# urw7rs/diffusion-models-made-easy

Hardware: AMD Instinct MI355X
Metric: denoising steps/sec + training images/sec, DDPM UNet CIFAR10 32×32 @1/2/4/8 GPU (higher is better)
Workload: dtype bf16; 1 GPU; DDPM T=1000 sampling, CIFAR10 32x32, default UNet (32,416,643 params, random init), batch 128 per GPU, t.shape=(1,); global_batch=128, parallelism=dp1 (independent chains per GPU, no data-path collective)

## Files before the change

diffusion-models-made-easy_amd/csrc/conv_thin.hip:

```cpp
#include <stdio.h>

#include <type_traits>

#include "conv_common.h"

namespace dmme {

constexpr int kThinMaxC = 512;

template <int NT, typename T = bf16, bool SPLIT = false>
__global__ void __launch_bounds__(256) conv_out_thin_kernel(ConvArgs a, int R) {
    typedef typename Vec8<T>::type bf16x8;
    extern __shared__ __attribute__((aligned(16))) char lds[];
    const int C = a.C1, W = a.Wout, H = a.Hout, NCOL = a.Cout * 9;
    float* par = reinterpret_cast<float*>(lds);
    float* z = par + 2 * C;
    constexpr int ZP = 32 * NT + 1;
    const int tid = threadIdx.x, lane = tid & 63, wave = tid >> 6;
    const int r = lane & 31, h = lane >> 5;
    const int bands = H / R, n = blockIdx.x / bands, y0 = (blockIdx.x % bands) * R;
    const int npx = (R + 2) * W, ntile = npx / 32;

    const int ksteps = C / 16;
    const T* wb = (const T*)a.w;
    bf16x8 wfrag[NT][8];
    bf16x8 wlo[SPLIT ? NT : 1][SPLIT ? 8 : 1];
    auto load_w = [&](int kc) __attribute__((always_inline)) {
#pragma unroll
        for (int t = 0; t < NT; ++t) {
            const int nc = 32 * t + r;
#pragma unroll
            for (int kg = 0; kg < 8; ++kg) {
                bf16x8 v, vl;
#pragma unroll
                for (int e = 0; e < 8; ++e) v[e] = vl[e] = (T)0.f;
                if constexpr (SPLIT) {
                    const int c0 = (kc + kg) * 16 + 8 * h;
                    if (kc + kg < ksteps && nc < NCOL) {
                        const T* wr = wb + (int64_t)nc * 2 * C + (c0 >> 5) * 64 + (c0 & 31);
                        v = *reinterpret_cast<const bf16x8*>(wr);
                        vl = *reinterpret_cast<const bf16x8*>(wr + 32);
                    }
                    wlo[t][kg] = vl;
                } else {
                    if (kc + kg < ksteps && nc < NCOL) v = *reinterpret_cast<const bf16x8*>(wb + (int64_t)nc * C + (kc + kg) * 16 + 8 * h);
                }
                wfrag[t][kg] = v;
            }
        }
    };
    const bool w_once = ksteps <= 8;
    if (w_once) load_w(0);
    for (int c = tid; c < C; c += 256) {
        float sc = 1.f, sh = 0.f;
        if (a.has_gni) {
            gn_in_scale_shift(a, n, c, C, y0 == 0, sc, sh);
        } else if (a.scale) {
            sc = a.scale[(int64_t)n * C + c];
            sh = a.shift[(int64_t)n * C + c];
        }
        par[c] = sc;
        par[C + c] = sh;
    }
    __syncthreads();

    typedef typename std::conditional<SPLIT, float, T>::type TX;
    const TX* xb = (const TX*)a.src1 + (int64_t)n * H * W * C;
    for (int tile = wave; tile < ntile; tile += 4) {
        const int p = tile * 32 + r;
        const int yy = y0 - 1 + p / W, xx = p % W;
        const bool in = yy >= 0 && yy < H;
        const TX* px = xb + (int64_t)((in ? yy : 0) * W + xx) * C + 8 * h;
        f32x16 acc[NT];
#pragma unroll
        for (int t = 0; t < NT; ++t)
#pragma unroll
            for (int j = 0; j < 16; ++j) acc[t][j] = 0.f;
        for (int kc = 0; kc < ksteps; kc += 8) {
            if (!w_once) load_w(kc);
            if constexpr (SPLIT) {
                uint4 raw[8][2];
#pragma unroll
                for (int kg = 0; kg < 8; ++kg)
                    if (kc + kg < ksteps) {
                        raw[kg][0] = *reinterpret_cast<const uint4*>(px + (kc + kg) * 16);
                        raw[kg][1] = *reinterpret_cast<const uint4*>(px + (kc + kg) * 16 + 4);
                    }
#pragma unroll
                for (int kg = 0; kg < 8; ++kg) {
                    if (kc + kg >= ksteps) break;
                    const int c0 = (kc + kg) * 16 + 8 * h;
                    bf16x8 ahi, alo;
#pragma unroll
                    for (int q = 0; q < 2; ++q) {
                        f32x4 y = __builtin_bit_cast(f32x4, raw[kg][q]);
                        if (a.scale) {
                            const f32x4 sc4 = *reinterpret_cast<const f32x4*>(par + c0 + 4 * q), sh4 = *reinterpret_cast<const f32x4*>(par + C + c0 + 4 * q);
#pragma unroll
                            for (int e = 0; e < 4; ++e) y[e] = fmaf(y[e], sc4[e], sh4[e]);
                        }
                        if (a.pro_silu) {
#pragma unroll
                            for (int e = 0; e < 4; ++e) y[e] = silu_fast(y[e]);
                        }
#pragma unroll
                        for (int e = 0; e < 4; ++e) {
                            const T hv = (T)(in ? y[e] : 0.f);
                            ahi[4 * q + e] = hv;
                            alo[4 * q + e] = (T)((in ? y[e] : 0.f) - (float)hv);
                        }
                    }
#pragma unroll
                    for (int t = 0; t < NT; ++t) {
                        mma16<T>(__builtin_bit_cast(uint4, alo), __builtin_bit_cast(uint4, wfrag[t][kg]), acc[t]);
                        mma16<T>(__builtin_bit_cast(uint4, ahi), __builtin_bit_cast(uint4, wlo[t][kg]), acc[t]);
                        mma16<T>(__builtin_bit_cast(uint4, ahi), __builtin_bit_cast(uint4, wfrag[t][kg]), acc[t]);
                    }
                }
            } else {
            uint4 raw[8];
#pragma unroll
            for (int kg = 0; kg < 8; ++kg)
                if (kc + kg < ksteps) raw[kg] = *reinterpret_cast<const uint4*>(px + (kc + kg) * 16);
#pragma unroll
            for (int kg = 0; kg < 8; ++kg) {
                if (kc + kg >= ksteps) break;
                const int c0 = (kc + kg) * 16 + 8 * h;
                uint4 av = prologue_vec<T>(raw[kg], a.scale ? par + c0 : nullptr, a.scale ? par + C + c0 : nullptr, nullptr, a.pro_silu);
                if (!in) av = make_uint4(0u, 0u, 0u, 0u);
#pragma unroll
                for (int t = 0; t < NT; ++t) mma16<T>(av, __builtin_bit_cast(uint4, wfrag[t][kg]), acc[t]);
            }
            }
        }
#pragma unroll
        for (int t = 0; t < NT; ++t)
#pragma unroll
            for (int j = 0; j < 16; ++j) z[(tile * 32 + (j & 3) + 8 * (j >> 2) + 4 * h) * ZP + 32 * t + r] = acc[t][j];
    }
    __syncthreads();
    const int hw = H * W;
    float* out = (float*)a.dst + (int64_t)n * a.Cout * hw;
    for (int q = tid; q < R * W; q += 256) {
        const int oy = q / W, ox = q % W;
        for (int k = 0; k < a.Cout; ++k) {
            float s = a.bias ? a.bias[k] : 0.f;
#pragma unroll
            for (int t9 = 0; t9 < 9; ++t9) {
                const int xs = ox + t9 % 3 - 1;
                if (xs < 0 || xs >= W) continue;
                s += z[((oy + t9 / 3) * W + xs) * ZP + k * 9 + t9];
            }
            out[(int64_t)k * hw + (y0 + oy) * W + ox] = s;
        }
    }
}

static int thin_rows(const ConvArgs& a) {
    const int NT = a.Cout * 9 <= 32 ? 1 : 2;
    const size_t cap = (a.mix == 3 ? 80 : 60) * 1024;
    for (int R = 16; R >= 2; R >>= 1)
        if (a.Hout % R == 0 && ((R + 2) * a.Wout) % 32 == 0 && (size_t)(R + 2) * a.Wout * (32 * NT + 1) * 4 + (size_t)2 * a.C1 * 4 <= cap &&
            (int64_t)a.N * (a.Hout / R) >= 512)
            return R;
    for (int R = 2; R <= 16; R <<= 1)
        if (a.Hout % R == 0 && ((R + 2) * a.Wout) % 32 == 0 && (size_t)(R + 2) * a.Wout * (32 * NT + 1) * 4 + (size_t)2 * a.C1 * 4 <= cap) return R;
    return 0;
}

bool conv_thin_route(int dtype, const ConvArgs& a, ConvRoute& r) {
    const bool off = getenv("DMME_NO_CONV_THIN") != nullptr;
    if (a.mix && a.mix != 3) return false;
    if (off || !is16(dtype) || a.x3) return false;
    if (a.mix == 3 && (dtype != DMME_F16 || a.C1 % 32)) return false;
    if (a.taps != 9 || a.stride != 1 || a.up || a.C2 || a.in_nchw || !a.out_nchw || a.out_silu || a.tproj || a.res1 || a.dmask || a.gn_part || a.n_gno)
        return false;
    if (a.Cout * 9 > 64 || a.C1 % 16 || a.C1 > kThinMaxC || a.Wout % 32 || a.Hin != a.Hout || a.Win != a.Wout) return false;
    if (thin_rows(a) <= 0) return false;
    r = make_route(CONV_THIN);
    return true;
}

int launch_conv_out_thin(const ConvArgs& a, hipStream_t s) {
    const int R = thin_rows(a);
    DMME_REQUIRE(R > 0, DMME_ERR_UNSUPPORTED, "conv_out_thin: unsupported shape");
    const int NT = a.Cout * 9 <= 32 ? 1 : 2;
    const size_t lds = (size_t)(R + 2) * a.Wout * (32 * NT + 1) * 4 + (size_t)2 * a.C1 * 4;
    const dim3 grid((unsigned)(a.N * (a.Hout / R)));
    if (a.mix == 3) {
        static bool attr = false;
        if (!attr) {
            DMME_CHECK_HIP(hipFuncSetAttribute(reinterpret_cast<const void*>(conv_out_thin_kernel<1, f16, true>), hipFuncAttributeMaxDynamicSharedMemorySize, 80 * 1024));
            DMME_CHECK_HIP(hipFuncSetAttribute(reinterpret_cast<const void*>(conv_out_thin_kernel<2, f16, true>), hipFuncAttributeMaxDynamicSharedMemorySize, 80 * 1024));
            attr = true;
        }
        if (NT == 1)
            hipLaunchKernelGGL((conv_out_thin_kernel<1, f16, true>), grid, dim3(256), lds, s, a, R);
        else
            hipLaunchKernelGGL((conv_out_thin_kernel<2, f16, true>), grid, dim3(256), lds, s, a, R);
    } else if (a.f16) {
        if (NT == 1)
            hipLaunchKernelGGL((conv_out_thin_kernel<1, f16>), grid, dim3(256), lds, s, a, R);
        else
            hipLaunchKernelGGL((conv_out_thin_kernel<2, f16>), grid, dim3(256), lds, s, a, R);
    } else if (NT == 1)
        hipLaunchKernelGGL((conv_out_thin_kernel<1, bf16>), grid, dim3(256), lds, s, a, R);
    else
        hipLaunchKernelGGL((conv_out_thin_kernel<2, bf16>), grid, dim3(256), lds, s, a, R);
    DMME_CHECK_LAUNCH();
    return DMME_OK;
}

}
```

diffusion-models-made-easy_amd/csrc/kernels_generic.hip:

```cpp
#include <stdlib.h>

#include <algorithm>

#include "common.h"

namespace dmme {

template <typename T>
__global__ void __launch_bounds__(256) conv_generic_kernel(ConvArgs a) {
    const int64_t total = (int64_t)a.N * a.Hout * a.Wout * a.Cout;
    const int Cin = a.C1 + a.C2;
    const int Hv = a.up ? 2 * a.Hin : a.Hin, Wv = a.up ? 2 * a.Win : a.Win;
    const int k = a.taps == 9 ? 3 : 1, pad = a.taps == 9 ? 1 : 0;
    for (int64_t idx = blockIdx.x * (int64_t)blockDim.x + threadIdx.x; idx < total;
         idx += (int64_t)gridDim.x * blockDim.x) {
        const int co = (int)(idx % a.Cout);
        int64_t p = idx / a.Cout;
        const int ow = (int)(p % a.Wout);
        p /= a.Wout;
        const int oh = (int)(p % a.Hout);
        const int n = (int)(p / a.Hout);
        const T* w = (const T*)a.w + (int64_t)co * a.taps * Cin;
        const float* sc = a.scale ? a.scale + (int64_t)n * Cin : nullptr;
        const float* sh = a.scale ? a.shift + (int64_t)n * Cin : nullptr;
        const float* dm = a.dmask ? a.dmask + (int64_t)n * Cin : nullptr;
        float acc = 0.f;
        for (int kh = 0; kh < k; ++kh) {
            const int iy = oh * a.stride - pad + kh;
            if (iy < 0 || iy >= Hv) continue;
            if (a.up == 2 && (iy & 1)) continue;
            const int sy = a.up ? (iy >> 1) : iy;
            for (int kw = 0; kw < k; ++kw) {
                const int ix = ow * a.stride - pad + kw;
                if (ix < 0 || ix >= Wv) continue;
                if (a.up == 2 && (ix & 1)) continue;
                const int sx = a.up ? (ix >> 1) : ix;
                const T* wt = w + (kh * k + kw) * Cin;
                const int64_t pix = ((int64_t)n * a.Hin + sy) * a.Win + sx;
                for (int ci = 0; ci < Cin; ++ci) {
                    float v;
                    if (a.in_nchw)
                        v = ((const float*)a.src1)[(((int64_t)n * a.C1 + ci) * a.Hin + sy) * a.Win + sx];
                    else if (ci < a.C1)
                        v = to_f(((const T*)a.src1)[pix * a.C1 + ci]);
                    else
                        v = to_f(((const T*)a.src2)[pix * a.C2 + (ci - a.C1)]);
                    if (sc) v = fmaf(v, sc[ci], sh[ci]);
                    if (a.pro_silu) v = silu_f(v);
                    if (dm) v *= dm[ci];
                    if (!a.in_nchw) v = to_f(from_f<T>(v));
                    acc = fmaf(v, to_f(wt[ci]), acc);
                }
            }
        }
        if (a.bias) acc += a.bias[co];
        if (a.tproj) acc += a.tproj[(int64_t)(a.nt == 1 ? 0 : n) * a.tproj_ld + co];
        const int64_t opix = ((int64_t)n * a.Hout + oh) * a.Wout + ow;
        if (a.res1) {
            if (co < a.R1)
                acc += to_f(((const T*)a.res1)[opix * a.R1 + co]);
            else
                acc += to_f(((const T*)a.res2)[opix * (a.Cout - a.R1) + (co - a.R1)]);
        }
        if (a.out_silu) acc = silu_f(acc);
        if (a.out_nchw)
            ((float*)a.dst)[(((int64_t)n * a.Cout + co) * a.Hout + oh) * a.Wout + ow] = acc;
        else
            ((T*)a.dst)[opix * a.Cout + co] = from_f<T>(acc);
    }
}

template <typename T>
__global__ void __launch_bounds__(256) conv_in_kernel(ConvArgs a, int px_per_block) {
    extern __shared__ __attribute__((aligned(16))) float wl[];
    const int Cin = a.C1, K = 9 * Cin, Cout = a.Cout;
    for (int e = threadIdx.x; e < K * Cout; e += blockDim.x) {
        const int co = e / K, k = e % K;
        wl[k * Cout + co] = to_f(((const T*)a.w)[e]);
    }
    __syncthreads();
    const int tpp = Cout / 8;
    const int ppb = 256 / tpp;
    const int cg = (threadIdx.x % tpp) * 8;
    const int64_t npix = (int64_t)a.N * a.Hout * a.Wout;
    const int64_t p0 = (int64_t)blockIdx.x * px_per_block;
    for (int pp = threadIdx.x / tpp; pp < px_per_block; pp += ppb) {
        const int64_t p = p0 + pp;
        if (p >= npix) break;
        const int ox = (int)(p % a.Wout), oy = (int)((p / a.Wout) % a.Hout), n = (int)(p / ((int64_t)a.Wout * a.Hout));
        float acc[8];
#pragma unroll
        for (int j = 0; j < 8; ++j) acc[j] = a.bias ? a.bias[cg + j] : 0.f;
        for (int kh = 0; kh < 3; ++kh) {
            const int iy = oy - 1 + kh;
            if (iy < 0 || iy >= a.Hin) continue;
            for (int kw = 0; kw < 3; ++kw) {
                const int ix = ox - 1 + kw;
                if (ix < 0 || ix >= a.Win) continue;
                for (int ci = 0; ci < Cin; ++ci) {
                    const float v = a.in_nchw ? ((const float*)a.src1)[(((int64_t)n * Cin + ci) * a.Hin + iy) * a.Win + ix]
                                              : to_f(((const T*)a.src1)[(((int64_t)n * a.Hin + iy) * a.Win + ix) * Cin + ci]);
                    const float* wr = wl + ((kh * 3 + kw) * Cin + ci) * Cout + cg;
                    const float4 w0 = *reinterpret_cast<const float4*>(wr), w1 = *reinterpret_cast<const float4*>(wr + 4);
                    acc[0] = fmaf(v, w0.x, acc[0]); acc[1] = fmaf(v, w0.y, acc[1]);
                    acc[2] = fmaf(v, w0.z, acc[2]); acc[3] = fmaf(v, w0.w, acc[3]);
                    acc[4] = fmaf(v, w1.x, acc[4]); acc[5] = fmaf(v, w1.y, acc[5]);
                    acc[6] = fmaf(v, w1.z, acc[6]); acc[7] = fmaf(v, w1.w, acc[7]);
                }
            }
        }
        T* o = (T*)a.dst + p * Cout + cg;
#pragma unroll
        for (int j = 0; j < 8; ++j) o[j] = from_f<T>(acc[j]);
    }
}

typedef float f32x16_g __attribute__((ext_vector_type(16)));
typedef float f32x4_g __attribute__((ext_vector_type(4)));
template <typename T, int CT>
__global__ void __launch_bounds__(256) conv_in_mfma_kernel(ConvArgs a, int nblocks) {
    const int lane = threadIdx.x & 63, r = lane & 31, h = lane >> 5;
    const int Cin = a.C1, K = 9 * Cin;
    float wreg[CT][14];
#pragma unroll
    for (int ct = 0; ct < CT; ++ct)
#pragma unroll
        for (int j = 0; j < 14; ++j) {
            const int k = 2 * j + h;
            wreg[ct][j] = k < K ? to_f(((const T*)a.w)[(int64_t)(ct * 32 + r) * K + k]) : 0.f;
        }
    const int HW = a.Hout * a.Wout;
    int t_off[14], t_dy[14], t_dx[14];
#pragma unroll
    for (int j = 0; j < 14; ++j) {
        const int k = 2 * j + h, tap = k / Cin, ci = k - tap * Cin;
        t_dy[j] = k < K ? tap / 3 - 1 : 1 << 20;
        t_dx[j] = tap % 3 - 1;
        t_off[j] = (ci * a.Hin + (tap / 3 - 1)) * a.Win + tap % 3 - 1;
    }
    __shared__ __attribute__((aligned(16))) float biasL[128];
    if (threadIdx.x < 32 * CT) biasL[threadIdx.x] = a.bias ? a.bias[threadIdx.x] : 0.f;
    __syncthreads();
    for (int blk = blockIdx.x * 4 + (threadIdx.x >> 6); blk < nblocks; blk += gridDim.x * 4) {
        const int p = blk * 32 + r;
        const int n = p / HW, rem = p - n * HW, oy = rem / a.Wout, ox = rem - oy * a.Wout;
        const float* xb = (const float*)a.src1 + ((int64_t)n * Cin * a.Hin + oy) * a.Win + ox;
        float xv[14];
#pragma unroll
        for (int j = 0; j < 14; ++j) {
            const bool in = (unsigned)(oy + t_dy[j]) < (unsigned)a.Hin && (unsigned)(ox + t_dx[j]) < (unsigned)a.Win;
            xv[j] = in ? xb[t_off[j]] : 0.f;
        }
        constexpr int PITCH = CT * 32 + 4;
        __shared__ __attribute__((aligned(16))) unsigned short stage_in[4][32 * PITCH];
        unsigned short* st = stage_in[threadIdx.x >> 6];
#pragma unroll
        for (int ct = 0; ct < CT; ++ct) {
            f32x16_g acc;
#pragma unroll
            for (int g4 = 0; g4 < 4; ++g4) {
                const f32x4_g b4 = *reinterpret_cast<const f32x4_g*>(biasL + ct * 32 + 8 * g4 + 4 * h);
                acc[4 * g4] = b4[0];
                acc[4 * g4 + 1] = b4[1];
                acc[4 * g4 + 2] = b4[2];
                acc[4 * g4 + 3] = b4[3];
            }
#pragma unroll
            for (int j = 0; j < 14; ++j) acc = __builtin_amdgcn_mfma_f32_32x32x2f32(wreg[ct][j], xv[j], acc, 0, 0, 0);
            if constexpr (sizeof(T) == 2) {
#pragma unroll
                for (int gq = 0; gq < 4; ++gq) {
                    typedef T bf16x4_g __attribute__((ext_vector_type(4)));
                    bf16x4_g v;
#pragma unroll
                    for (int e = 0; e < 4; ++e) v[e] = (T)acc[4 * gq + e];
                    *reinterpret_cast<bf16x4_g*>(st + r * PITCH + ct * 32 + 8 * gq + 4 * h) = v;
                    if (a.gn_part) {
                        float s = 0.f, ss = 0.f;
#pragma unroll
                        for (int e = 0; e < 4; ++e) {
                            const float x = (float)v[e];
                            s += x;
                            ss = fmaf(x, x, ss);
                        }
                        s = half_sum(s);
                        ss = half_sum(ss);
                        if (r == 0) {
                            const float mean = s * (1.f / 128.f);
                            float* po = a.gn_part + (((int64_t)n * a.gn_tiles + (rem >> 5)) * (a.Cout / 4) + ct * 8 + 2 * gq + h) * 2;
                            po[0] = mean;
                            po[1] = ss - s * mean;
                        }
                    }
                }
            } else {
                T* o = (T*)a.dst + (int64_t)p * a.Cout + ct * 32 + 4 * h;
#pragma unroll
                for (int gq = 0; gq < 4; ++gq)
                    *reinterpret_cast<float4*>(o + 8 * gq) = make_float4(acc[4 * gq], acc[4 * gq + 1], acc[4 * gq + 2], acc[4 * gq + 3]);
                if (a.gn_part) {
#pragma unroll
                    for (int gq = 0; gq < 4; ++gq) {
                        float s = 0.f, ss = 0.f;
#pragma unroll
                        for (int e = 0; e < 4; ++e) {
                            const float x = acc[4 * gq + e];
                            s += x;
                            ss = fmaf(x, x, ss);
                        }
                        s = half_sum(s);
                        ss = half_sum(ss);
                        if (r == 0) {
                            const float mean = s * (1.f / 128.f);
                            float* po = a.gn_part + (((int64_t)n * a.gn_tiles + (rem >> 5)) * (a.Cout / 4) + ct * 8 + 2 * gq + h) * 2;
                            po[0] = mean;
                            po[1] = ss - s * mean;
                        }
                    }
                }
            }
        }
        if constexpr (sizeof(T) == 2) {
            __builtin_amdgcn_wave_barrier();
            constexpr int VPR = CT * 4;
#pragma unroll
            for (int q = 0; q < 32 * VPR / 64; ++q) {
                const int it = lane + 64 * q, px = it / VPR, sg = it % VPR;
                const uint2 lo = *reinterpret_cast<const uint2*>(st + px * PITCH + sg * 8), hi = *reinterpret_cast<const uint2*>(st + px * PITCH + sg * 8 + 4);
                *reinterpret_cast<uint4*>((T*)a.dst + (int64_t)(blk * 32 + px) * a.Cout + sg * 8) = make_uint4(lo.x, lo.y, hi.x, hi.y);
            }
            __builtin_amdgcn_wave_barrier();
        }
    }
}

static bool conv_in_mfma_supported(const ConvArgs& a) {
    return a.in_nchw && !a.out_nchw && a.taps == 9 && a.stride == 1 && !a.up && a.C2 == 0 && a.C1 <= 3 && !a.scale && !a.pro_silu && !a.dmask &&
           !a.tproj && !a.res1 && !a.out_silu && (a.Cout == 128 || a.Cout == 64 || a.Cout == 32) &&
           (!a.gn_part || (a.gn_cg == 4 && (a.Hout * a.Wout) % 32 == 0)) &&
           ((int64_t)a.N * a.Hout * a.Wout) % 32 == 0 && (int64_t)a.N * a.Hout * a.Wout * a.Cout < (1ll << 31) && !debug_route("no_conv_in_mfma");
}

void conv_generic_route(const ConvArgs& a, ConvRoute& r) {
    r = make_route(CONV_GENERIC);
    if (!conv_in_mfma_supported(a) || (a.Hout * a.Wout) % 32) return;
    r.vec = r.stat_bn = 4;
    r.stat_px = 32;
    r.stat_tiles = a.Hout * a.Wout / 32;
}

static bool conv_in_supported(const ConvArgs& a) {
    return !a.out_nchw && a.taps == 9 && a.stride == 1 && !a.up && a.C2 == 0 && a.C1 <= 8 && !a.scale &&
           !a.pro_silu && !a.dmask && !a.tproj && !a.res1 && !a.out_silu && a.Cout % 8 == 0 && a.Cout <= 2048 &&
           256 % (a.Cout / 8) == 0 && (size_t)9 * a.C1 * a.Cout * 4 <= 48 * 1024;
}

const char* conv_generic_kernel_name(const ConvArgs& a) {
    return conv_in_mfma_supported(a) ? "conv_in_mfma_kernel" : conv_in_supported(a) ? "conv_in_kernel" : "conv_generic_kernel";
}

int launch_conv_generic(int dtype, const ConvArgs& a, hipStream_t s) {
    if (conv_in_mfma_supported(a)) {
        const int nblocks = (int)((int64_t)a.N * a.Hout * a.Wout / 32);
        unsigned grid = (unsigned)((nblocks + 3) / 4);
        if (grid > 512u) grid = 512u;
#define DMME_CIN(TT, CT) hipLaunchKernelGGL((conv_in_mfma_kernel<TT, CT>), dim3(grid), dim3(256), 0, s, a, nblocks)
        if (dtype == DMME_BF16) {
            if (a.Cout == 128) DMME_CIN(bf16, 4); else if (a.Cout == 64) DMME_CIN(bf16, 2); else DMME_CIN(bf16, 1);
        } else if (dtype == DMME_F16) {
            if (a.Cout == 128) DMME_CIN(f16, 4); else if (a.Cout == 64) DMME_CIN(f16, 2); else DMME_CIN(f16, 1);
        } else {
            if (a.Cout == 128) DMME_CIN(float, 4); else if (a.Cout == 64) DMME_CIN(float, 2); else DMME_CIN(float, 1);
        }
#undef DMME_CIN
        DMME_CHECK_LAUNCH();
        return DMME_OK;
    }
    if (conv_in_supported(a) && !a.gn_part) {
        const int64_t npix = (int64_t)a.N * a.Hout * a.Wout;
        const int ppb = 256 / (a.Cout / 8) * 8;
        const unsigned blocks = (unsigned)((npix + ppb - 1) / ppb);
        const size_t lds = (size_t)9 * a.C1 * a.Cout * 4;
        if (dtype == DMME_BF16)
            hipLaunchKernelGGL(conv_in_kernel<bf16>, dim3(blocks), dim3(256), lds, s, a, ppb);
        else if (dtype == DMME_F16)
            hipLaunchKernelGGL(conv_in_kernel<f16>, dim3(blocks), dim3(256), lds, s, a, ppb);
        else
            hipLaunchKernelGGL(conv_in_kernel<float>, dim3(blocks), dim3(256), lds, s, a, ppb);
        DMME_CHECK_LAUNCH();
        return DMME_OK;
    }
    const int64_t total = (int64_t)a.N * a.Hout * a.Wout * a.Cout;
    if (total == 0) return DMME_OK;
    int64_t blocks = (total + 255) / 256;
    if (blocks > 65536) blocks = 65536;
    if (dtype == DMME_BF16)
        hipLaunchKernelGGL(conv_generic_kernel<bf16>, dim3((unsigned)blocks), dim3(256), 0, s, a);
    else if (dtype == DMME_F16)
        hipLaunchKernelGGL(conv_generic_kernel<f16>, dim3((unsigned)blocks), dim3(256), 0, s, a);
    else
        hipLaunchKernelGGL(conv_generic_kernel<float>, dim3((unsigned)blocks), dim3(256), 0, s, a);
    DMME_CHECK_LAUNCH();
    return DMME_OK;
}

template <typename T>
__global__ void __launch_bounds__(256) gn_generic_kernel(const T* __restrict__ s1, const T* __restrict__ s2, int HW,
                                                         int C1, int C2, int groups, const float* gamma,
                                                         const float* beta, float eps, float* scale, float* shift,
                                                         float* mean_rstd) {
    __shared__ float red[16];
    const int n = blockIdx.y, g = blockIdx.x;
    const int C = C1 + C2, cg = C / groups;
    const int64_t cnt = (int64_t)cg * HW;
    auto at = [&](int64_t e) -> float {
        const int c = g * cg + (int)(e % cg);
        const int64_t p = (int64_t)n * HW + e / cg;
        return c < C1 ? to_f(s1[p * C1 + c]) : to_f(s2[p * C2 + (c - C1)]);
    };
    float s = 0.f;
    for (int64_t e = threadIdx.x; e < cnt; e += blockDim.x) s += at(e);
    const float mean = block_sum(s, red) / (float)cnt;
    float q = 0.f;
    for (int64_t e = threadIdx.x; e < cnt; e += blockDim.x) {
        const float d = at(e) - mean;
        q = fmaf(d, d, q);
    }
    const float var = block_sum(q, red) / (float)cnt;
    const float rstd = 1.0f / sqrtf(var + eps);
    if (mean_rstd && threadIdx.x == 0) {
        mean_rstd[((int64_t)n * groups + g) * 2] = mean;
        mean_rstd[((int64_t)n * groups + g) * 2 + 1] = rstd;
    }
    for (int j = threadIdx.x; j < cg; j += blockDim.x) {
        const int c = g * cg + j;
        const float a = rstd * gamma[c];
        scale[(int64_t)n * C + c] = a;
        shift[(int64_t)n * C + c] = beta[c] - mean * a;
    }
}

int launch_gn_generic(int dtype, const void* src1, const void* src2, int N, int HW, int C1, int C2, int groups,
                      const float* gamma, const float* beta, float eps, float* scale, float* shift, float* mean_rstd,
                      hipStream_t s) {
    dim3 grid(groups, N);
    if (dtype == DMME_BF16)
        hipLaunchKernelGGL(gn_generic_kernel<bf16>, grid, dim3(256), 0, s, (const bf16*)src1, (const bf16*)src2, HW,
                           C1, C2, groups, gamma, beta, eps, scale, shift, mean_rstd);
    else if (dtype == DMME_F16)
        hipLaunchKernelGGL(gn_generic_kernel<f16>, grid, dim3(256), 0, s, (const f16*)src1, (const f16*)src2, HW,
                           C1, C2, groups, gamma, beta, eps, scale, shift, mean_rstd);
    else
        hipLaunchKernelGGL(gn_generic_kernel<float>, grid, dim3(256), 0, s, (const float*)src1, (const float*)src2,
                           HW, C1, C2, groups, gamma, beta, eps, scale, shift, mean_rstd);
    DMME_CHECK_LAUNCH();
    return DMME_OK;
}

template <typename T>
__global__ void __launch_bounds__(256) attn_generic_kernel(const T* __restrict__ qkv, int S, int C, int heads, int N, T* __restrict__ out) {
    extern __shared__ __attribute__((aligned(16))) float sm[];
    const int d = C / heads;
    float* qs = sm;
    float* ps = sm + d;
    float* red = ps + S;
    const int bh = blockIdx.y, n = bh / heads, hd = bh % heads, i = blockIdx.x;
    const T* base = qkv + (int64_t)n * S * 3 * C + (int64_t)hd * 3 * d;
    const float kscale = powf((float)C, -0.5f);
    for (int c = threadIdx.x; c < d; c += blockDim.x) qs[c] = to_f(base[(int64_t)i * 3 * C + c]);
    __syncthreads();
    float lmax = -INFINITY;
    for (int j = threadIdx.x; j < S; j += blockDim.x) {
        const T* kr = base + (int64_t)j * 3 * C + d;
        float acc = 0.f;
        for (int c = 0; c < d; ++c) acc = fmaf(qs[c], to_f(from_f<T>(to_f(kr[c]) * kscale)), acc);
        ps[j] = acc;
        lmax = fmaxf(lmax, acc);
    }
    const float m = block_max(lmax, red);
    float lsum = 0.f;
    for (int j = threadIdx.x; j < S; j += blockDim.x) {
        const float e = expf(ps[j] - m);
        ps[j] = e;
        lsum += e;
    }
    const float tot = block_sum(lsum, red);
    __syncthreads();
    const float inv = 1.0f / tot;
    const int on = bh % N, oh = bh / N;
    for (int c = threadIdx.x; c < d; c += blockDim.x) {
        float acc = 0.f;
        for (int j = 0; j < S; ++j) acc = fmaf(to_f(from_f<T>(ps[j] * inv)), to_f(base[(int64_t)j * 3 * C + 2 * d + c]), acc);
        out[((int64_t)on * S + i) * C + oh * d + c] = from_f<T>(acc);
    }
}

template <typename T>
__global__ void __launch_bounds__(256) attn_s16_kernel(const T* __restrict__ qkv, int C, int heads, int N, T* __restrict__ out) {
    extern __shared__ __attribute__((aligned(16))) float sm[];
    constexpr int S = 16;
    const int d = C / heads, dp = d + 4;
    float* qs = sm;
    float* ks = qs + S * dp;
    float* vs = ks + S * dp;
    float* ps = vs + S * dp;
    const int bh = blockIdx.x, n = bh / heads, hd = bh % heads, tid = threadIdx.x;
    const T* base = qkv + (int64_t)n * S * 3 * C + (int64_t)hd * 3 * d;
    const float kscale = powf((float)C, -0.5f);
    for (int e = tid; e < S * d; e += 256) {
        const int row = e / d, c = e - row * d;
        const T* p = base + (int64_t)row * 3 * C + c;
        qs[row * dp + c] = to_f(p[0]);
        ks[row * dp + c] = to_f(from_f<T>(to_f(p[d]) * kscale));
        vs[row * dp + c] = to_f(p[2 * d]);
    }
    __syncthreads();
    const int i = tid >> 4, j = tid & 15;
    float acc = 0.f;
    for (int c = 0; c < d; c += 4) {
        const f32x4_g a = *reinterpret_cast<const f32x4_g*>(qs + i * dp + c), b = *reinterpret_cast<const f32x4_g*>(ks + j * dp + c);
        acc = fmaf(a[0], b[0], acc);
        acc = fmaf(a[1], b[1], acc);
        acc = fmaf(a[2], b[2], acc);
        acc = fmaf(a[3], b[3], acc);
    }
    float m = acc;
    m = fmaxf(m, DMME_DPP_F(m, 0xB1));
    m = fmaxf(m, DMME_DPP_F(m, 0x4E));
    m = fmaxf(m, DMME_DPP_F(m, 0x141));
    m = fmaxf(m, DMME_DPP_F(m, 0x140));
    const float e = expf(acc - m);
    const float tot = row16_sum(e);
    ps[i * 17 + j] = to_f(from_f<T>(e * (1.0f / tot)));
    __syncthreads();
    const int on = bh % N, oh = bh / N;
    for (int c = j; c < d; c += 16) {
        float o = 0.f;
#pragma unroll
        for (int jj = 0; jj < S; ++jj) o = fmaf(ps[i * 17 + jj], vs[jj * dp + c], o);
        out[((int64_t)on * S + i) * C + oh * d + c] = from_f<T>(o);
    }
}

int launch_attn_heads(int dtype, const void* qkv, int N, int S, int C, int heads, void* out, hipStream_t s) {
    DMME_REQUIRE(heads >= 1 && C % heads == 0, DMME_ERR_INVALID, "attention: width %d not divisible by %d heads", C, heads);
    if (S == 16 && (C / heads) % 4 == 0 && C / heads <= 1024 && !debug_route("no_attn_s16")) {
        const size_t lds16 = (size_t)(3 * 16 * (C / heads + 4) + 16 * 17) * sizeof(float);
        if (lds16 <= 64 * 1024) {
            if (dtype == DMME_BF16)
                hipLaunchKernelGGL(attn_s16_kernel<bf16>, dim3((unsigned)(N * heads)), dim3(256), lds16, s, (const bf16*)qkv, C, heads, N, (bf16*)out);
            else if (dtype == DMME_F16)
                hipLaunchKernelGGL(attn_s16_kernel<f16>, dim3((unsigned)(N * heads)), dim3(256), lds16, s, (const f16*)qkv, C, heads, N, (f16*)out);
            else
                hipLaunchKernelGGL(attn_s16_kernel<float>, dim3((unsigned)(N * heads)), dim3(256), lds16, s, (const float*)qkv, C, heads, N, (float*)out);
            DMME_CHECK_LAUNCH();
            return DMME_OK;
        }
    }
    const size_t lds = (size_t)(C / heads + S + 16) * sizeof(float);
    DMME_REQUIRE(lds <= 64 * 1024, DMME_ERR_UNSUPPORTED, "attention generic: d+S too large (%d+%d)", C / heads, S);
    dim3 grid(S, N * heads);
    if (dtype == DMME_BF16)
        hipLaunchKernelGGL(attn_generic_kernel<bf16>, grid, dim3(256), lds, s, (const bf16*)qkv, S, C, heads, N, (bf16*)out);
    else if (dtype == DMME_F16)
        hipLaunchKernelGGL(attn_generic_kernel<f16>, grid, dim3(256), lds, s, (const f16*)qkv, S, C, heads, N, (f16*)out);
    else
        hipLaunchKernelGGL(attn_generic_kernel<float>, grid, dim3(256), lds, s, (const float*)qkv, S, C, heads, N, (float*)out);
    DMME_CHECK_LAUNCH();
    return DMME_OK;
}
int launch_attn_generic(int dtype, const void* qkv, int N, int S, int C, void* out, hipStream_t s) {
    return launch_attn_heads(dtype, qkv, N, S, C, 1, out, s);
}

__global__ void gn_modulate_kernel(float* __restrict__ scale, float* __restrict__ shift, const float* __restrict__ t_shift,
                                   const float* __restrict__ t_scale, int ld, int nt, int N, int C) {
    const int i = blockIdx.x * blockDim.x + threadIdx.x;
    if (i >= N * C) return;
    const int n = i / C, c = i % C, r = nt == 1 ? 0 : n;
    const float m = 1.0f + t_scale[(int64_t)r * ld + c];
    scale[i] = scale[i] * m;
    shift[i] = fmaf(shift[i], m, t_shift[(int64_t)r * ld + c]);
}
int launch_gn_modulate(float* scale, float* shift, const float* t_shift, const float* t_scale, int ld, int nt, int N, int C, hipStream_t s) {
    hipLaunchKernelGGL(gn_modulate_kernel, dim3((N * C + 255) / 256), dim3(256), 0, s, scale, shift, t_shift, t_scale, ld, nt, N, C);
    DMME_CHECK_LAUNCH();
    return DMME_OK;
}

__global__ void time_sinusoid_kernel(const int64_t* t, int nt, const float* freqs, int half, float* out, unsigned* mark, unsigned mark_val) {
    const int i = blockIdx.x * blockDim.x + threadIdx.x;
    if (i == 0 && mark) *mark = mark_val;
    if (i >= nt * half) return;
    const int r = i / half, k = i % half;
    const float arg = (float)t[r] * freqs[k];
    out[(int64_t)r * 2 * half + k] = sinf(arg);
    out[(int64_t)r * 2 * half + half + k] = cosf(arg);
}

int launch_time_sinusoid(const int64_t* t, int nt, const float* freqs, int half, float* out, hipStream_t s, unsigned* mark, unsigned mark_val) {
    const int total = nt * half;
    hipLaunchKernelGGL(time_sinusoid_kernel, dim3((total + 255) / 256), dim3(256), 0, s, t, nt, freqs, half, out, mark, mark_val);
    DMME_CHECK_LAUNCH();
    return DMME_OK;
}

__global__ void __launch_bounds__(256) label_cond_kernel(const float* z2, int nt, const float* __restrict__ E, const int64_t* __restrict__ labels, int K,
                                                         int emb, float* __restrict__ temb, float* zsave, int* status) {
    const int b = blockIdx.x;
    const int64_t y = labels[b];
    const bool ok = y >= 0 && y <= (int64_t)K;
    const int row = y < 0 ? 0 : (y > (int64_t)K ? K : (int)y);
    const float* zr = z2 + (int64_t)(nt == 1 ? 0 : b) * emb;
    const float* er = E + (int64_t)row * emb;
    for (int c = threadIdx.x; c < emb; c += blockDim.x) {
        const float v = zr[c] + er[c];
        if (zsave) zsave[(int64_t)b * emb + c] = v;
        temb[(int64_t)b * emb + c] = ok ? silu_f(v) : NAN;
    }
    if (!ok && threadIdx.x == 0 && status) atomicExch(status, 1);
}
int launch_label_cond(const float* z2, int nt, const float* E, const int64_t* labels, int B, int K, int emb, float* temb, float* zsave, int* status,
                      hipStream_t s) {
    DMME_REQUIRE(z2 && E && labels && temb && B > 0 && K >= 1 && emb > 0 && (nt == 1 || nt == B), DMME_ERR_INVALID, "label_cond: bad argument");
    DMME_REQUIRE(!zsave || zsave != z2 || nt == B, DMME_ERR_INVALID, "label_cond: in-place pre-activations need one time row per image");
    hipLaunchKernelGGL(label_cond_kernel, dim3((unsigned)B), dim3(256), 0, s, z2, nt, E, labels, K, emb, temb, zsave, status);
    DMME_CHECK_LAUNCH();
    return DMME_OK;
}

__global__ void __launch_bounds__(256) label_grad_kernel(const float* __restrict__ dz2, const int64_t* __restrict__ labels, int B, int emb,
                                                         float* __restrict__ dE) {
    __shared__ unsigned char hit[256];
    const int64_t k = blockIdx.x;
    const int tid = threadIdx.x;
    for (int c0 = 0; c0 < emb; c0 += 256) {
        const int c = c0 + tid;
// ... 573 lines not shown
```

Baseline: 469.6 denoising steps/s (one step = UNet forward + DDPM update on a batch of 128), summed over GPUs.

## Prefetch next input gather and stage conv_in weights through LDS

Restructures the first-layer conv MFMA kernel so each wave gathers the input pixels for its next block while computing the current one, giving a software-pipelined loop. Weights are now loaded with coalesced vector loads into shared memory and then scattered into registers, replacing strided per-thread global loads. Boundary checks use a precomputed tap bitmask. Optional compile-time clock-stamp instrumentation is also added to both kernels; it is disabled by default. The trade-off is higher register pressure from the double-buffered input and an extra barrier, and the shared buffer is reused for both weights and the output stage.

New measurement: 470.8 denoising steps/s (one step = UNet forward + DDPM update on a batch of 128), summed over GPUs (median of 6 runs). No clear change (+0.3%).

```diff
diff --git a/diffusion-models-made-easy_amd/csrc/conv_thin.hip b/diffusion-models-made-easy_amd/csrc/conv_thin.hip
--- a/diffusion-models-made-easy_amd/csrc/conv_thin.hip
+++ b/diffusion-models-made-easy_amd/csrc/conv_thin.hip
@@ -8,6 +8,13 @@
 
 constexpr int kThinMaxC = 512;
 
+#ifdef THIN_STAMPS
+#define THIN_STAMP() { __builtin_amdgcn_sched_barrier(0); if (stamping && st_i < 64) st_lds[st_i++] = (long long)clock64(); __builtin_amdgcn_sched_barrier(0); }
+#define THIN_STAMP_W() { __builtin_amdgcn_sched_barrier(0); __builtin_amdgcn_s_waitcnt(0); THIN_STAMP(); }
+#else
+#define THIN_STAMP()
+#define THIN_STAMP_W()
+#endif
 template <int NT, typename T = bf16, bool SPLIT = false>
 __global__ void __launch_bounds__(256) conv_out_thin_kernel(ConvArgs a, int R) {
     typedef typename Vec8<T>::type bf16x8;
@@ -50,6 +57,12 @@
         }
     };
     const bool w_once = ksteps <= 8;
+#ifdef THIN_STAMPS
+    __shared__ long long st_lds[64];
+    int st_i = 0;
+    const bool stamping = a.stamps && blockIdx.x == 0 && tid == 0;
+#endif
+    THIN_STAMP();
     if (w_once) load_w(0);
     for (int c = tid; c < C; c += 256) {
         float sc = 1.f, sh = 0.f;
@@ -63,6 +76,7 @@
         par[C + c] = sh;
     }
     __syncthreads();
+    THIN_STAMP();
 
     typedef typename std::conditional<SPLIT, float, T>::type TX;
     const TX* xb = (const TX*)a.src1 + (int64_t)n * H * W * C;
@@ -122,6 +136,7 @@
 #pragma unroll
             for (int kg = 0; kg < 8; ++kg)
                 if (kc + kg < ksteps) raw[kg] = *reinterpret_cast<const uint4*>(px + (kc + kg) * 16);
+            THIN_STAMP();
 #pragma unroll
             for (int kg = 0; kg < 8; ++kg) {
                 if (kc + kg >= ksteps) break;
@@ -133,12 +148,15 @@
             }
             }
         }
+        THIN_STAMP();
 #pragma unroll
         for (int t = 0; t < NT; ++t)
 #pragma unroll
             for (int j = 0; j < 16; ++j) z[(tile * 32 + (j & 3) + 8 * (j >> 2) + 4 * h) * ZP + 32 * t + r] = acc[t][j];
+        THIN_STAMP();
     }
     __syncthreads();
+    THIN_STAMP();
     const int hw = H * W;
     float* out = (float*)a.dst + (int64_t)n * a.Cout * hw;
     for (int q = tid; q < R * W; q += 256) {
@@ -154,7 +172,15 @@
             out[(int64_t)k * hw + (y0 + oy) * W + ox] = s;
         }
     }
-}
+    THIN_STAMP();
+    THIN_STAMP_W();
+#ifdef THIN_STAMPS
+    if (stamping)
+        for (int i = 0; i < st_i; ++i) a.stamps[i] = st_lds[i];
+#endif
+}
+#undef THIN_STAMP
+#undef THIN_STAMP_W
 
 static int thin_rows(const ConvArgs& a) {
     const int NT = a.Cout * 9 <= 32 ? 1 : 2;
diff --git a/diffusion-models-made-easy_amd/csrc/kernels_generic.hip b/diffusion-models-made-easy_amd/csrc/kernels_generic.hip
--- a/diffusion-models-made-easy_amd/csrc/kernels_generic.hip
+++ b/diffusion-models-made-easy_amd/csrc/kernels_generic.hip
@@ -117,43 +117,113 @@
 
 typedef float f32x16_g __attribute__((ext_vector_type(16)));
 typedef float f32x4_g __attribute__((ext_vector_type(4)));
+template <int CIN>
+__device__ __forceinline__ void cin_tap_table(int h, int Hin, int Win, int (&t_off)[14], int (&t_tap)[14]) {
+#pragma unroll
+    for (int j = 0; j < 14; ++j) {
+        int off[2], tp[2];
+#pragma unroll
+        for (int e = 0; e < 2; ++e) {
+            const int k = 2 * j + e, tap = k / CIN, ci = k % CIN;
+            off[e] = k < 9 * CIN ? (ci * Hin + (tap / 3 - 1)) * Win + tap % 3 - 1 : 0;
+            tp[e] = k < 9 * CIN ? tap : 31;
+        }
+        t_off[j] = h ? off[1] : off[0];
+        t_tap[j] = h ? tp[1] : tp[0];
+    }
+}
+#ifdef CIN_STAMPS
+#define CIN_STAMP() { __builtin_amdgcn_sched_barrier(0); if (stamping && st_i < 64) st_lds[st_i++] = (long long)clock64(); __builtin_amdgcn_sched_barrier(0); }
+#define CIN_STAMP_W() { __builtin_amdgcn_sched_barrier(0); __builtin_amdgcn_s_waitcnt(0); CIN_STAMP(); }
+#else
+#define CIN_STAMP()
+#define CIN_STAMP_W()
+#endif
 template <typename T, int CT>
 __global__ void __launch_bounds__(256) conv_in_mfma_kernel(ConvArgs a, int nblocks) {
     const int lane = threadIdx.x & 63, r = lane & 31, h = lane >> 5;
     const int Cin = a.C1, K = 9 * Cin;
-    float wreg[CT][14];
-#pragma unroll
-    for (int ct = 0; ct < CT; ++ct)
+    constexpr int PITCH = CT * 32 + 4;
+    constexpr int STAGE_BYTES = sizeof(T) == 2 ? 4 * 32 * PITCH * 2 : 0, W_BYTES = CT * 32 * 27 * (int)sizeof(T);
+    __shared__ __attribute__((aligned(16))) unsigned char smem[STAGE_BYTES > W_BYTES ? STAGE_BYTES : W_BYTES];
+    __shared__ __attribute__((aligned(16))) float biasL[128];
+#ifdef CIN_STAMPS
+    __shared__ long long st_lds[64];
+    int st_i = 0;
+    const bool stamping = a.stamps && blockIdx.x == 0 && threadIdx.x == 0;
+#endif
+    CIN_STAMP();
+    int t_off[14], t_tap[14];
+    if (Cin == 3) cin_tap_table<3>(h, a.Hin, a.Win, t_off, t_tap);
+    else if (Cin == 2) cin_tap_table<2>(h, a.Hin, a.Win, t_off, t_tap);
+    else cin_tap_table<1>(h, a.Hin, a.Win, t_off, t_tap);
+    const int HW = a.Hout * a.Wout;
+    auto gather = [&](int b, float (&x)[14], int& n_, int& rem_) __attribute__((always_inline)) {
+        const int p = b * 32 + r;
+        n_ = p / HW;
+        rem_ = p - n_ * HW;
+        const int oy = rem_ / a.Wout, ox = rem_ - oy * a.Wout;
+        const float* xb = (const float*)a.src1 + ((int64_t)n_ * Cin * a.Hin + oy) * a.Win + ox;
+        const unsigned cm = (ox > 0 ? 1u : 0u) | 2u | (ox + 1 < a.Win ? 4u : 0u);
+        const unsigned mask = (oy > 0 ? cm : 0u) | cm << 3 | (oy + 1 < a.Hin ? cm << 6 : 0u);
 #pragma unroll
         for (int j = 0; j < 14; ++j) {
-            const int k = 2 * j + h;
-            wreg[ct][j] = k < K ? to_f(((const T*)a.w)[(int64_t)(ct * 32 + r) * K + k]) : 0.f;
-        }
-    const int HW = a.Hout * a.Wout;
-    int t_off[14], t_dy[14], t_dx[14];
-#pragma unroll
-    for (int j = 0; j < 14; ++j) {
-        const int k = 2 * j + h, tap = k / Cin, ci = k - tap * Cin;
-        t_dy[j] = k < K ? tap / 3 - 1 : 1 << 20;
-        t_dx[j] = tap % 3 - 1;
-        t_off[j] = (ci * a.Hin + (tap / 3 - 1)) * a.Win + tap % 3 - 1;
-    }
-    __shared__ __attribute__((aligned(16))) float biasL[128];
+            const bool in = (mask >> t_tap[j]) & 1u;
+            const float v = xb[in ? t_off[j] : 0];
+            x[j] = in ? v : 0.f;
+        }
+    };
+    const int bstep = gridDim.x * 4;
+    int blk = blockIdx.x * 4 + (threadIdx.x >> 6);
+    float xv[14];
+    int n = 0, rem = 0;
+#pragma unroll
+    for (int j = 0; j < 14; ++j) xv[j] = 0.f;
+    if (blk < nblocks) gather(blk, xv, n, rem);
+    {
+        const T* wg = (const T*)a.w;
+        const int nw = CT * 32 * K;
+        if ((reinterpret_cast<uintptr_t>(wg) & 15) == 0) {
+            const int nv = nw * (int)sizeof(T) / 16;
+            constexpr int NIT = (W_BYTES / 16 + 255) / 256;
+            uint4 wv[NIT];
+#pragma unroll
+            for (int it = 0; it < NIT; ++it) {
+                const int v = threadIdx.x + 256 * it;
+                wv[it] = reinterpret_cast<const uint4*>(wg)[v < nv ? v : 0];
+            }
+#pragma unroll
+            for (int it = 0; it < NIT; ++it) {
+                const int v = threadIdx.x + 256 * it;
+                if (v < nv) reinterpret_cast<uint4*>(smem)[v] = wv[it];
+            }
+        } else {
+#pragma clang loop vectorize(disable) unroll(disable)
+            for (int e = threadIdx.x; e < nw; e += 256) reinterpret_cast<T*>(smem)[e] = wg[e];
+        }
+    }
     if (threadIdx.x < 32 * CT) biasL[threadIdx.x] = a.bias ? a.bias[threadIdx.x] : 0.f;
     __syncthreads();
-    for (int blk = blockIdx.x * 4 + (threadIdx.x >> 6); blk < nblocks; blk += gridDim.x * 4) {
-        const int p = blk * 32 + r;
-        const int n = p / HW, rem = p - n * HW, oy = rem / a.Wout, ox = rem - oy * a.Wout;
-        const float* xb = (const float*)a.src1 + ((int64_t)n * Cin * a.Hin + oy) * a.Win + ox;
-        float xv[14];
-#pragma unroll
-        for (int j = 0; j < 14; ++j) {
-            const bool in = (unsigned)(oy + t_dy[j]) < (unsigned)a.Hin && (unsigned)(ox + t_dx[j]) < (unsigned)a.Win;
-            xv[j] = in ? xb[t_off[j]] : 0.f;
-        }
-        constexpr int PITCH = CT * 32 + 4;
-        __shared__ __attribute__((aligned(16))) unsigned short stage_in[4][32 * PITCH];
-        unsigned short* st = stage_in[threadIdx.x >> 6];
+    float wreg[CT][14];
+#pragma unroll
+    for (int j = 0; j < 14; ++j) {
+        const int k = 2 * j + h;
+#pragma unroll
+        for (int ct = 0; ct < CT; ++ct) {
+            const float wv = to_f(reinterpret_cast<const T*>(smem)[(ct * 32 + r) * K + (k < K ? k : 0)]);
+            wreg[ct][j] = k < K ? wv : 0.f;
+        }
+    }
+    __syncthreads();
+    CIN_STAMP();
+    for (; blk < nblocks; blk += bstep) {
+        float xn[14];
+        int nn = 0, remn = 0;
+#pragma unroll
+        for (int j = 0; j < 14; ++j) xn[j] = 0.f;
+        if (blk + bstep < nblocks) gather(blk + bstep, xn, nn, remn);
+        CIN_STAMP();
+        unsigned short* st = reinterpret_cast<unsigned short*>(smem) + (threadIdx.x >> 6) * 32 * PITCH;
 #pragma unroll
         for (int ct = 0; ct < CT; ++ct) {
             f32x16_g acc;
@@ -167,6 +237,7 @@
             }
 #pragma unroll
             for (int j = 0; j < 14; ++j) acc = __builtin_amdgcn_mfma_f32_32x32x2f32(wreg[ct][j], xv[j], acc, 0, 0, 0);
+            if (ct == 0) CIN_STAMP();
             if constexpr (sizeof(T) == 2) {
 #pragma unroll
                 for (int gq = 0; gq < 4; ++gq) {
@@ -194,7 +265,7 @@
                     }
                 }
             } else {
-                T* o = (T*)a.dst + (int64_t)p * a.Cout + ct * 32 + 4 * h;
+                T* o = (T*)a.dst + (int64_t)(blk * 32 + r) * a.Cout + ct * 32 + 4 * h;
 #pragma unroll
                 for (int gq = 0; gq < 4; ++gq)
                     *reinterpret_cast<float4*>(o + 8 * gq) = make_float4(acc[4 * gq], acc[4 * gq + 1], acc[4 * gq + 2], acc[4 * gq + 3]);
@@ -220,6 +291,7 @@
                 }
             }
         }
+        CIN_STAMP();
         if constexpr (sizeof(T) == 2) {
             __builtin_amdgcn_wave_barrier();
             constexpr int VPR = CT * 4;
@@ -231,8 +303,20 @@
             }
             __builtin_amdgcn_wave_barrier();
         }
-    }
-}
+        CIN_STAMP();
+#pragma unroll
+        for (int j = 0; j < 14; ++j) xv[j] = xn[j];
+        n = nn;
+        rem = remn;
+    }
+    CIN_STAMP_W();
+#ifdef CIN_STAMPS
+    if (stamping)
+        for (int i = 0; i < st_i; ++i) a.stamps[i] = st_lds[i];
+#endif
+}
+#undef CIN_STAMP
+#undef CIN_STAMP_W
 
 static bool conv_in_mfma_supported(const ConvArgs& a) {
     return a.in_nchw && !a.out_nchw && a.taps == 9 && a.stride == 1 && !a.up && a.C2 == 0 && a.C1 <= 3 && !a.scale && !a.pro_silu && !a.dmask &&
```
